# ath92/splat-renderer

Hardware: AMD Instinct MI355X
Metric: Msplats/sec (higher is better)
Workload: dtype f32

## Files before the change

### include/splat.h

```cpp
#ifndef SPLAT_H
#define SPLAT_H

#include <stddef.h>
#include <stdint.h>

#ifdef __cplusplus
extern "C" {
#endif

#define SPLAT_ABI_VERSION 3

#define SPLAT_OK 0
#define SPLAT_ERR_INVALID (-1)
#define SPLAT_ERR_HIP (-2)
#define SPLAT_ERR_OOM (-3)
#define SPLAT_ERR_CAPACITY (-4)
#define SPLAT_ERR_STATE (-5)
#define SPLAT_ERR_NO_DEVICE (-6)
#define SPLAT_ERR_COMM (-7)
#define SPLAT_ERR_RETRY (-8)

typedef struct splat_ctx splat_ctx;
typedef struct splat_sorter splat_sorter;
typedef struct splat_binner splat_binner;
// ... 17 lines not shown

int splat_ctx_create(int device_ordinal, splat_ctx **out);
int splat_ctx_create_on_stream(int device_ordinal, void *hip_stream, splat_ctx **out);
void splat_ctx_destroy(splat_ctx *ctx);
const char *splat_last_error(splat_ctx *ctx);
int splat_sync(splat_ctx *ctx);
int splat_abi_version(void);
int splat_set_timing(splat_ctx *ctx, int enabled);
#define SPLAT_TIMING_COUNT_ENTRIES 0x80000000u
int splat_set_timing_stages(splat_ctx *ctx, uint32_t stage_mask);
int splat_set_timing_sampling(splat_ctx *ctx, uint32_t every);
int splat_stage_time_ms(splat_ctx *ctx, int stage, float *ms);
int splat_stage_time_stats(splat_ctx *ctx, int stage, uint32_t *samples, double *total_ms);
int splat_timing_consumed(splat_ctx *ctx, uint64_t *staged, uint64_t *consumed);

int splat_buf_alloc(splat_ctx *ctx, size_t bytes, void **dptr);
int splat_buf_free(splat_ctx *ctx, void *dptr);
int splat_buf_upload(splat_ctx *ctx, void *dst_dptr, const void *src_host, size_t bytes);
int splat_buf_download(splat_ctx *ctx, void *dst_host, const void *src_dptr, size_t bytes);
int splat_buf_zero(splat_ctx *ctx, void *dptr, size_t bytes);
int splat_buf_copy(splat_ctx *ctx, void *dst_dptr, const void *src_dptr, size_t bytes);

int splat_update_props(splat_ctx *ctx, const void *positions, const void *curvature, uint32_t n,
                       void *props);
int splat_update_props_planes(splat_ctx *ctx, const void *positions, const void *curvature, uint32_t n,
                              void *pos_radius, void *color_opacity);
int splat_props_to_planes(splat_ctx *ctx, const void *props, uint32_t n, void *pos_radius, void *color_opacity);

int splat_project(splat_ctx *ctx, const float *uniforms, const void *pos_radius,
                  uint32_t pr_stride_vec4, uint32_t n, void *projected, void *keys, void *payload,
                  uint32_t n_padded);

int splat_extract_keys(splat_ctx *ctx, const void *projected, uint32_t n, uint32_t n_padded,
                       void *keys, void *payload);

int splat_sort_create(splat_ctx *ctx, uint32_t capacity, splat_sorter **out);
void splat_sort_destroy(splat_sorter *s);
uint32_t splat_sort_capacity(const splat_sorter *s);
void *splat_sort_keys(splat_sorter *s);
void *splat_sort_payload(splat_sorter *s);
int splat_sort_run(splat_sorter *s, uint32_t n, uint32_t bit_begin, uint32_t bit_end);
void *splat_sort_sorted_payload(splat_sorter *s);
void *splat_sort_sorted_keys(splat_sorter *s);
int splat_probe_lds_atomic_order(splat_ctx *ctx, uint64_t *mismatches);
int splat_sort_set_mode(splat_sorter *s, int mode);
int splat_rank_status(splat_ctx *ctx, int *policy, int *atomics_ordered, uint32_t *order_faults);
#ifdef SPLAT_TEST_HOOKS
int splat_debug_inject_order_fault(splat_ctx *ctx, uint32_t tile, uint32_t position);
int splat_debug_set_tile_order(splat_ctx *ctx, const void *order_dptr);
int splat_debug_set_tile_sort_order(splat_ctx *ctx, const void *order_dptr);
int splat_debug_rerun_tile_sort(splat_ctx *ctx, splat_binner *binner);
int splat_debug_tile_sort_launches(splat_ctx *ctx, uint32_t *launches);
int splat_debug_lds_rate(splat_ctx *ctx, int kind, uint32_t workgroups_per_cu, uint32_t iters, float *ms);
#endif
int splat_composite_forget_history(splat_ctx *ctx);
int splat_composite_options(splat_ctx *ctx, int kernel, int ahead, int predict);

int splat_scan_u32(splat_ctx *ctx, const void *in, void *out, uint32_t n, void *total_dptr);

int splat_bin_create(splat_ctx *ctx, uint32_t tile_size, splat_binner **out);
void splat_bin_destroy(splat_binner *b);
int splat_bin_run(splat_binner *b, const void *projected, uint32_t n_splats, const void *sorted,
                  uint32_t n_sorted, uint32_t width, uint32_t height, uint32_t tile_row0,
                  uint32_t tile_row1);
uint32_t splat_bin_tile_size(const splat_binner *b);
int splat_bin_counts(splat_binner *b, void **dptr);
int splat_bin_offsets(splat_binner *b, void **dptr);
int splat_bin_indices(splat_binner *b, void **dptr);
int splat_bin_total(splat_binner *b, uint64_t *total_pairs);
#define SPLAT_FRAME_ORDER_DEFAULT (-1)
#define SPLAT_FRAME_SORT_FIRST 0
#define SPLAT_FRAME_TILE_FIRST 1
int splat_bin_set_frame_order(splat_binner *b, int order);
int splat_bin_dims(splat_binner *b, uint32_t *ntx, uint32_t *nty);

int splat_validate_tile_order(splat_ctx *ctx, const void *projected, const void *tile_offsets,
                              uint32_t num_tiles, const void *tile_indices, uint64_t total_pairs,
                              uint64_t *violations_host);

#define SPLAT_COMPOSITE_FRONT_TO_BACK 0
#define SPLAT_COMPOSITE_REFERENCE_LITERAL 1
#define SPLAT_RECORDS_PROJECTED 0
#define SPLAT_RECORDS_COMPACT 1
#define SPLAT_RECORDS_DISC48 2
#define SPLAT_RECORDS_LIT32 3
#define SPLAT_FOOTPRINT_ISOTROPIC 0
#define SPLAT_FOOTPRINT_DISC 1
#define SPLAT_FOOTPRINT_ELLIPSOID 2
typedef struct splat_composite_cfg {
    uint32_t mode;
    uint32_t early_out;
    uint32_t tile_size;
    uint32_t tile_row0;
    uint32_t tile_row1;
    uint32_t record_format;
    uint32_t prelit;
    uint32_t footprint;
} splat_composite_cfg;
int splat_lit_colors(splat_ctx *ctx, const void *color_opacity, uint32_t color_stride_vec4,
                     const void *normals, uint32_t normal_stride_vec4, uint32_t n, void *lit);
int splat_composite(splat_ctx *ctx, const splat_composite_cfg *cfg, const void *color_opacity,
                    uint32_t color_stride_vec4, const void *normals, uint32_t normal_stride_vec4,
                    const void *projected, const void *tile_indices, const void *tile_counts,
                    const void *tile_offsets, uint32_t width, uint32_t height, void *out_rgba8,
                    void *out_rgba32f, void *consumed_dptr);

// ... 245 lines not shown
```

### splat_renderer_amd/_lib.py

```python
import ctypes as C
import os

_HERE = os.path.dirname(os.path.abspath(__file__))
LIB_PATH = os.environ.get("SPLAT_LIB_PATH") or os.path.join(_HERE, "libsplat_hip.so")

OK = 0
ERR_NAMES = {-1: "INVALID", -2: "HIP", -3: "OOM", -4: "CAPACITY", -5: "STATE", -6: "NO_DEVICE", -7: "COMM", -8: "RETRY"}
ERR_CAPACITY, ERR_RETRY = -4, -8
RENDER_AGAIN = (ERR_CAPACITY, ERR_RETRY)

STAGE_PROJECT, STAGE_SORT, STAGE_BIN, STAGE_COMPOSITE, STAGE_EXCHANGE, STAGE_BIN_SCATTER, STAGE_BIN_PASS2, STAGE_BIN_TILE_SORT = range(8)
STAGE_NAMES = ("project", "sort", "bin", "composite", "exchange", "bin_scatter", "bin_second_pass", "bin_tile_sort")
TIMING_COUNT_ENTRIES = 0x80000000
MODE_FRONT_TO_BACK, MODE_REFERENCE_LITERAL = 0, 1
RECORDS_PROJECTED, RECORDS_COMPACT, RECORDS_DISC48, RECORDS_LIT32 = 0, 1, 2, 3
FOOTPRINT_ISOTROPIC, FOOTPRINT_DISC, FOOTPRINT_ELLIPSOID = 0, 1, 2
U32_MAX = 0xFFFFFFFF


class SplatError(RuntimeError):
    def __init__(self, code, msg):
        super().__init__(f"libsplat_hip error {ERR_NAMES.get(code, code)}: {msg}")
        self.code = code

# ... 128 lines not shown
    "splat_bin_destroy": (None, [_vp]),
    "splat_bin_run": (_i, [_vp, _vp, _u32, _vp, _u32, _u32, _u32, _u32, _u32]),
    "splat_bin_tile_size": (_u32, [_vp]),
    "splat_bin_counts": (_i, [_vp, _pvp]),
    "splat_bin_offsets": (_i, [_vp, _pvp]),
    "splat_bin_indices": (_i, [_vp, _pvp]),
    "splat_bin_total": (_i, [_vp, C.POINTER(C.c_uint64)]),
    "splat_bin_set_frame_order": (_i, [_vp, _i]),
    "splat_bin_dims": (_i, [_vp, C.POINTER(_u32), C.POINTER(_u32)]),
    "splat_validate_tile_order": (_i, [_vp, _vp, _vp, _u32, _vp, C.c_uint64, C.POINTER(C.c_uint64)]),
    "splat_lit_colors": (_i, [_vp, _vp, _u32, _vp, _u32, _u32, _vp]),
    "splat_composite": (_i, [_vp, C.POINTER(CompositeCfg), _vp, _u32, _vp, _u32, _vp, _vp, _vp, _vp, _u32, _u32,
                             _vp, _vp, _vp]),
    "splat_render_frame": (_i, [_vp, _vp, _vp, C.POINTER(CompositeCfg), C.POINTER(C.c_float), _vp, _vp, _u32, _u32,
                                _u32, _vp, _vp, _vp]),
    "splat_render_frame_planes": (_i, [_vp, _vp, _vp, C.POINTER(CompositeCfg), C.POINTER(C.c_float), _vp, _vp, _vp, _u32,
                                       _u32, _u32, _vp, _vp, _vp]),
    "splat_composite_aov": (_i, [_vp, C.POINTER(CompositeCfg), _vp, _u32, _vp, _u32, _vp, _vp, _vp, _vp, _u32, _u32,
                                 _vp, _vp, _vp, C.POINTER(Aov)]),
    "splat_render_frame_aov": (_i, [_vp, _vp, _vp, C.POINTER(CompositeCfg), C.POINTER(C.c_float), _vp, _vp, _u32, _u32,
                                    _u32, _vp, _vp, _vp, C.POINTER(Aov)]),
    "splat_render_frame_planes_aov": (_i, [_vp, _vp, _vp, C.POINTER(CompositeCfg), C.POINTER(C.c_float), _vp, _vp, _vp,
                                           _u32, _u32, _u32, _vp, _vp, _vp, C.POINTER(Aov)]),
    "splat_project_slice": (_i, [_vp, C.POINTER(C.c_float), _vp, _u32, _u32, _u32, _vp]),
    "splat_project_slice_compact": (_i, [_vp, C.POINTER(C.c_float), _vp, _u32, _u32, _u32, _vp]),
    "splat_project_slice_disc": (_i, [_vp, C.POINTER(C.c_float), _vp, _u32, _vp, _u32, _u32, _u32, _vp]),
    "splat_expand_compact": (_i, [_vp, _vp, _u32, _u32, _vp]),
    "splat_band_frame": (_i, [_vp, _vp, _vp, C.POINTER(CompositeCfg), _vp, _vp, _vp, _u32, _u32, _u32, _vp, _vp, _vp]),
    "splat_band_settle": (_i, [_vp, _vp, _vp, C.POINTER(_u32), C.POINTER(C.c_uint64)]),
    "splat_band_kept": (_i, [_vp, _vp, C.POINTER(_u32)]),
    "splat_band_keys": (_i, [_vp, _vp, _vp, _u32, _u32, _u32, _u32, _u32, _u32, C.POINTER(_u32)]),
    "splat_sdf_gradients": (_i, [_vp, _vp, _u32, _vp, _u32, _vp]),
    "splat_sdf_update_positions": (_i, [_vp, _vp, _vp, _u32, _vp]),
    "splat_sdf_scale_factors": (_i, [_vp, _vp, _u32, _vp, _u32, _vp]),
    "splat_sdf_curvature": (_i, [_vp, _vp, _vp, _u32, _vp]),
    "splat_sdf_seed_positions": (_i, [_vp, C.POINTER(C.c_float), C.POINTER(C.c_float), _u32, C.c_uint64, _vp]),
    "splat_sdf_generate": (_i, [_vp, _vp, _u32, C.POINTER(C.c_float), C.POINTER(C.c_float), C.c_uint64, _vp, _u32, _u32, _vp, _vp, _vp, _vp]),
    "splat_point_frame": (_i, [_vp, _vp, C.POINTER(C.c_float), _vp, _u32, _vp, _u32, _vp, _u32, _u32, _u32, _u32, _vp, _vp, _vp, _vp]),
    "splat_comm_unique_id": (_i, [_vp]),
    "splat_comm_init": (_i, [_vp, _i, _i, _vp, _pvp]),
    "splat_comm_destroy": (None, [_vp]),
    "splat_comm_rank": (_i, [_vp, C.POINTER(_i), C.POINTER(_i)]),
    "splat_comm_count": (_i, [_vp, C.POINTER(_i), C.POINTER(_i)]),
    "splat_allgather_records": (_i, [_vp, _vp, _vp, _vp, _sz]),
}
COMM_ID_BYTES = 128
HOOK_SIGNATURES = {
    "splat_debug_inject_order_fault": (_i, [_vp, _u32, _u32]),
    "splat_debug_set_tile_order": (_i, [_vp, _vp]),
    "splat_debug_set_tile_sort_order": (_i, [_vp, _vp]),
    "splat_debug_rerun_tile_sort": (_i, [_vp, _vp]),
    "splat_debug_tile_sort_launches": (_i, [_vp, C.POINTER(_u32)]),
    "splat_debug_lds_rate": (_i, [_vp, _i, _u32, _u32, C.POINTER(C.c_float)]),
}
HOOKS_LIB_PATH = os.path.join(_HERE, "libsplat_hip_hooks.so")

_lib = None


class _Bound:

    def __getattr__(self, name):
        if name in HOOK_SIGNATURES:
            raise AttributeError(f"libsplat_hip: {name} is a test hook: the shipped library does not carry it; run with "
                                 f"SPLAT_LIB_PATH={HOOKS_LIB_PATH} (the -DSPLAT_TEST_HOOKS build)")
        raise AttributeError(f"libsplat_hip: {name} is not declared in splat_renderer_amd._lib.SIGNATURES")


def load():
    global _lib
    if _lib is not None:
        return _lib
    if not os.path.exists(LIB_PATH):
        raise ImportError(
            f"{LIB_PATH} not found: build it with `python -c 'import __graft_entry__ as g; g.build()'` "
            "(hipcc --offload-arch=gfx950). splat_renderer_amd has no CPU fallback.")
    dll = C.CDLL(LIB_PATH)
    lib = _Bound()
    for name, (res, args) in SIGNATURES.items():
        fn = getattr(dll, name)
        fn.restype = res
        fn.argtypes = args
        setattr(lib, name, fn)
    lib.has_hooks = hasattr(dll, "splat_debug_inject_order_fault")
    if lib.has_hooks:
        for name, (res, args) in HOOK_SIGNATURES.items():
            fn = getattr(dll, name)
            fn.restype = res
            fn.argtypes = args
            setattr(lib, name, fn)
    lib._dll = dll
    _lib = lib
    return lib


def check(rc, ctx=None):
    if rc != OK:
        msg = load().splat_last_error(ctx)
        raise SplatError(rc, msg.decode("utf-8", "replace") if msg else "")
    return rc
```

### splat_renderer_amd/csrc/project.hip

```cpp
#include "common.h"
#include "variant.h"
#include "tile_range.h"
#include "block_scan.h"
#include "disc.h"
#include "ellipsoid.h"
#include "shade.h"

struct FrameUniforms {
    float m[16];
    float eye[3];
    float time;
    float w, h;
};

__device__ __forceinline__ void to_screen(const FrameUniforms &u, float x, float y, float z, float &sx, float &sy) {
    float cx = ((u.m[0] * x + u.m[4] * y) + u.m[8] * z) + u.m[12];
    float cy = ((u.m[1] * x + u.m[5] * y) + u.m[9] * z) + u.m[13];
    float cw = ((u.m[3] * x + u.m[7] * y) + u.m[11] * z) + u.m[15];
    float nx = cx / cw, ny = cy / cw;
    sx = ((nx + 1.0f) * 0.5f) * u.w;
    sy = ((1.0f - ny) * 0.5f) * u.h;
}

__device__ __forceinline__ uint32_t depth_key(float depth) {
    uint32_t bits = __float_as_uint(depth);
    uint32_t mask = ((bits >> 31) == 1u) ? 0xffffffffu : 0x80000000u;
    return bits ^ mask;
}

__device__ __forceinline__ float4 project_centre(const FrameUniforms &u, float4 pr) {
    float x = pr.x, y = pr.y, z = pr.z, radius = pr.w;
    float dx = x - u.eye[0], dy = y - u.eye[1], dz = z - u.eye[2];
    float depth = sqrtf((dx * dx + dy * dy) + dz * dz);
    float scx, scy;
    to_screen(u, x, y, z, scx, scy);
    float max_d2 = 0.0f;
#pragma unroll
    for (int k = 0; k < 6; ++k) {
        float ox = (k == 0) ? radius : (k == 1) ? -radius : 0.0f;
        float oy = (k == 2) ? radius : (k == 3) ? -radius : 0.0f;
        float oz = (k == 4) ? radius : (k == 5) ? -radius : 0.0f;
        float sx, sy;
        to_screen(u, x + ox, y + oy, z + oz, sx, sy);
        float ex = scx - sx, ey = scy - sy;
        max_d2 = fmaxf(max_d2, ex * ex + ey * ey);
    }
    const float max_r = sqrtf(max_d2);
    return make_float4(scx, scy, max_r, depth);
}

struct DiscIO {
    const float4 *normals;
    uint32_t normal_stride;
    float4 *discs;
    uint32_t disc_stride;
    EllIO ell;
};

template <bool BALL>
__device__ __forceinline__ bool cannot_reach_band(const FrameUniforms &u, float4 pr, float r, const BinParams &bp) {
    const float *m = u.m;
    const float cx = ((m[0] * pr.x + m[4] * pr.y) + m[8] * pr.z) + m[12];
    const float cy = ((m[1] * pr.x + m[5] * pr.y) + m[9] * pr.z) + m[13];
    const float cw = ((m[3] * pr.x + m[7] * pr.y) + m[11] * pr.z) + m[15];
    const float ax = r * (BALL ? 1.001f * __builtin_amdgcn_sqrtf((m[0] * m[0] + m[4] * m[4]) + m[8] * m[8])
                               : fmaxf(fmaxf(fabsf(m[0]), fabsf(m[4])), fabsf(m[8])));
    const float ay = r * (BALL ? 1.001f * __builtin_amdgcn_sqrtf((m[1] * m[1] + m[5] * m[5]) + m[9] * m[9])
                               : fmaxf(fmaxf(fabsf(m[1]), fabsf(m[5])), fabsf(m[9])));
    const float aw = r * (BALL ? 1.001f * __builtin_amdgcn_sqrtf((m[3] * m[3] + m[7] * m[7]) + m[11] * m[11])
                               : fmaxf(fmaxf(fabsf(m[3]), fabsf(m[7])), fabsf(m[11])));
    const float den = cw - aw;
    if (!(cw > 0.0f) || !(den > 0.0f)) return false;
    const float icw = __builtin_amdgcn_rcpf(cw), iden = __builtin_amdgcn_rcpf(den);
    const float ndx = cx * icw, ndy = cy * icw;
    const float bx = (0.5f * u.w) * (ax + fabsf(ndx) * aw) * iden, by = (0.5f * u.h) * (ay + fabsf(ndy) * aw) * iden;
    const float reach = __builtin_amdgcn_sqrtf(bx * bx + by * by) * (1.5f * 1.001f) + 1.0f;
    const float scy = ((1.0f - ndy) * 0.5f) * u.h;
    const float ts = (float)bp.tile;
    return (scy + reach < (float)bp.row0 * ts - 2.0f) || (scy - reach > (float)bp.row1 * ts + 2.0f);
}

struct SplatIn {
    float4 pr, col, nrm, scl, rot;
};
template <bool DISC, bool LIT, bool ELL = false>
__device__ __forceinline__ SplatIn load_splat(const float4 *__restrict__ pos_radius, uint32_t stride_vec4, uint32_t i, const DiscIO &dio,
                                              const LitIO &lio) {
    SplatIn s;
    s.pr = pos_radius[(size_t)i * stride_vec4];
    s.col = s.nrm = s.scl = s.rot = make_float4(0.0f, 0.0f, 0.0f, 0.0f);
    if (ELL) {
        s.scl = dio.ell.scales[(size_t)i * dio.ell.scale_stride];
        s.rot = dio.ell.rotations[(size_t)i * dio.ell.rot_stride];
    } else if (DISC) s.nrm = dio.normals[(size_t)i * dio.normal_stride];
    if (LIT) {
        s.col = lio.color[(size_t)i * lio.color_stride];
        if (!lio.prelit) s.nrm = lio.normals[(size_t)i * lio.normal_stride];
    }
    return s;
}

template <bool WITH_KEYS, bool WITH_RANGE, bool DISC, bool LIT = false, bool WIDE = false, bool ELL = false>
__device__ __forceinline__ uint32_t project_one(const FrameUniforms &u, const SplatIn &in, uint32_t i, uint32_t index_base,
                                                float4 *__restrict__ projected, uint32_t *__restrict__ keys,
                                                uint32_t *__restrict__ payload, uint32_t *__restrict__ range32, const BinParams &bp,
                                                const DiscIO &dio, const LitIO &lio = LitIO{}, uint32_t kslot = 0xffffffffu) {
    const uint32_t ks = kslot == 0xffffffffu ? i : kslot;
    float4 a, b;
    float depth;
    if (DISC) {
        const float4 pr = in.pr;
        const DiscRecord d = ELL ? ellipsoid_record(u.m, u.w, u.h, pr, in.scl, in.rot) : disc_record(u.m, u.w, u.h, pr, in.nrm);
        dio.discs[(size_t)i * dio.disc_stride] = d.a;
        dio.discs[(size_t)i * dio.disc_stride + 1] = d.b;
        const float dx = pr.x - u.eye[0], dy = pr.y - u.eye[1], dz = pr.z - u.eye[2];
        depth = sqrtf((dx * dx + dy * dy) + dz * dz);
        if (LIT) {
            const float4 lc = (ELL || lio.prelit) ? in.col : lit_color(in.col, in.nrm);
            dio.discs[(size_t)i * dio.disc_stride + 2] = make_float4(lc.x, lc.y, lc.z, depth);
        }
        disc_bounds(d, a);
        b = make_float4(depth, 0.5f * fmaxf(a.z - a.x, a.w - a.y), __uint_as_float(index_base + i), 0.0f);
    } else {
        const float4 c = project_centre(u, in.pr);
        const float scx = c.x, scy = c.y, max_r = c.z;
        depth = c.w;
        float padded = max_r * 1.5f;
        a = make_float4(scx - padded, scy - padded, scx + padded, scy + padded);
        b = make_float4(depth, max_r, __uint_as_float(index_base + i), 0.0f);
        if (LIT) {
            lio.records[(size_t)i * 2] = c;
            lio.records[(size_t)i * 2 + 1] = lio.prelit ? in.col : lit_color(in.col, in.nrm);
        }
    }
    if ((!DISC && !LIT) || projected) {
        projected[(size_t)i * 2] = a;
        projected[(size_t)i * 2 + 1] = b;
    }
    if (WITH_KEYS) {
        keys[ks] = depth_key(depth);
        if (payload) payload[ks] = index_base + i;
    }
    uint32_t packed = 1u;
    if (WITH_RANGE) {
        uint32_t tx0, tx1, ty0, ty1;
        const bool ok = tile_range(a, bp.width, bp.height, bp.tile, bp.ntx, bp.nty, bp.row0, bp.row1, tx0, tx1, ty0, ty1);
        if (WIDE) {
            reinterpret_cast<uint2 *>(range32)[ks] = pack_range_wide(ok, tx0, tx1, ty0, ty1);
        } else {
            packed = pack_range32(ok, tx0, tx1, ty0, ty1);
            range32[ks] = packed;
        }
    }
    return packed;
}

__global__ __launch_bounds__(256) void k_project_compact(FrameUniforms u, const float4 *__restrict__ pos_radius, uint32_t stride_vec4,
                                                         uint32_t n, float4 *__restrict__ records16) {
    const uint32_t i = blockIdx.x * 256u + threadIdx.x;
    if (i < n) records16[i] = project_centre(u, pos_radius[(size_t)i * stride_vec4]);
}

__global__ __launch_bounds__(256) void k_project_disc48(FrameUniforms u, const float4 *__restrict__ pos_radius, uint32_t stride_vec4,
                                                        const float4 *__restrict__ normals, uint32_t normal_stride, uint32_t n,
                                                        float4 *__restrict__ records48) {
    const uint32_t i = blockIdx.x * 256u + threadIdx.x;
    if (i >= n) return;
    const float4 pr = pos_radius[(size_t)i * stride_vec4];
    const DiscRecord d = disc_record(u.m, u.w, u.h, pr, normals[(size_t)i * normal_stride]);
    const float dx = pr.x - u.eye[0], dy = pr.y - u.eye[1], dz = pr.z - u.eye[2];
    records48[(size_t)i * 3] = d.a;
    records48[(size_t)i * 3 + 1] = d.b;
    records48[(size_t)i * 3 + 2] = make_float4(sqrtf((dx * dx + dy * dy) + dz * dz), 0.0f, 0.0f, 0.0f);
}

__global__ __launch_bounds__(256) void k_expand_compact(const float4 *__restrict__ records16, uint32_t n, uint32_t index_base,
                                                        float4 *__restrict__ projected) {
    const uint32_t i = blockIdx.x * 256u + threadIdx.x;
    if (i >= n) return;
    const float4 c = records16[i];
    const float padded = c.z * 1.5f;
    projected[(size_t)i * 2] = make_float4(c.x - padded, c.y - padded, c.x + padded, c.y + padded);
    projected[(size_t)i * 2 + 1] = make_float4(c.w, c.z, __uint_as_float(index_base + i), 0.0f);
}

template <bool WITH_KEYS, bool WITH_RANGE, bool DISC, bool LIT = false, bool ELL = false>
__global__ __launch_bounds__(256) void k_project(FrameUniforms u, const float4 *__restrict__ pos_radius,
                                                 uint32_t stride_vec4, uint32_t n, uint32_t n_padded, uint32_t index_base,
                                                 float4 *__restrict__ projected, uint32_t *__restrict__ keys,
                                                 uint32_t *__restrict__ payload, uint32_t *__restrict__ range32, BinParams bp,
                                                 DiscIO dio, LitIO lio) {
    uint32_t i = blockIdx.x * 256u + threadIdx.x;
    if (i >= n) {
        if (WITH_KEYS && i < n_padded) {
            keys[i] = 0xffffffffu;
            if (payload) payload[i] = 0xffffffffu;
        }
        return;
    }
    const SplatIn in = load_splat<DISC, LIT, ELL>(pos_radius, stride_vec4, i, dio, lio);
    project_one<WITH_KEYS, WITH_RANGE, DISC, LIT, false, ELL>(u, in, i, index_base, projected, keys, payload, range32, bp, dio, lio);
}

template <bool DISC, bool LIT, bool ELL = false>
__global__ __launch_bounds__(256) void k_project_wide(FrameUniforms u, const float4 *__restrict__ pos_radius, uint32_t stride_vec4,
                                                      uint32_t n, uint32_t n_padded, float4 *__restrict__ projected,
                                                      uint32_t *__restrict__ keys, uint2 *__restrict__ range_wide, BinParams bp,
                                                      DiscIO dio, LitIO lio) {
    const uint32_t i = blockIdx.x * 256u + threadIdx.x;
    if (i >= n) {
        if (i < n_padded) keys[i] = 0xffffffffu;
        return;
    }
    const SplatIn in = load_splat<DISC, LIT, ELL>(pos_radius, stride_vec4, i, dio, lio);
    project_one<true, true, DISC, LIT, true, ELL>(u, in, i, 0, projected, keys, nullptr, reinterpret_cast<uint32_t *>(range_wide), bp, dio,
                                                  lio);
}

template <bool DISC, bool LIT, uint32_t PER, uint32_t AHEAD = 1, bool ELL = false>
__global__ __launch_bounds__(256) void k_project_hist(FrameUniforms u, const float4 *__restrict__ pos_radius, uint32_t stride_vec4,
                                                      uint32_t n, uint32_t n_padded, float4 *__restrict__ projected,
                                                      uint32_t *__restrict__ keys, uint32_t *__restrict__ range32, BinParams bp,
                                                      TfHistOut ho, DiscIO dio, LitIO lio) {
    __shared__ uint32_t lh[4][256];
    __shared__ uint32_t wsum[4];
    const uint32_t tid = threadIdx.x, w = tid >> 6;
    const uint32_t blk = xcd_block_of(blockIdx.x, ho.xcd_per);
    if (blk * (PER * 256u) >= n_padded) return;
    SplatIn in[PER];
#pragma unroll
    for (uint32_t k = 0; k < AHEAD; ++k) {
        const uint32_t i = blk * (PER * 256u) + k * 256u + tid;
        if (i < n) in[k] = load_splat<DISC, LIT, ELL>(pos_radius, stride_vec4, i, dio, lio);
    }
    if (blk == 0 && tid == 0) *ho.overflow_flag = 0;
    for (uint32_t j = tid; j < 4 * 256; j += 256) (&lh[0][0])[j] = 0;
    __syncthreads();
    uint32_t local = 0;
#pragma unroll
    for (uint32_t k = 0; k < PER; ++k) {
        if (k + AHEAD < PER) {
            const uint32_t i = blk * (PER * 256u) + (k + AHEAD) * 256u + tid;
            if (i < n) in[k + AHEAD] = load_splat<DISC, LIT, ELL>(pos_radius, stride_vec4, i, dio, lio);
        }
        const uint32_t i = blk * (PER * 256u) + k * 256u + tid;
        if (i >= n) {
            if (i < n_padded) keys[i] = 0xffffffffu;
            continue;
        }
        const uint32_t r = project_one<true, true, DISC, LIT, false, ELL>(u, in[k], i, 0, projected, keys, nullptr, range32, bp, dio, lio);
        const TileRect t = unpack_range32(r);
        if (t.empty()) continue;
        local += hist_add_rect(lh[w], t, bp.ntx, ho.mask);
    }
    local = wave_sum(local);
    if ((tid & 63) == 0) wsum[w] = local;
    __syncthreads();
    if (blk < ho.num_parts) {
        hist_flush<4>(lh, ho.hist, ho.num_parts, blk, ho.mask);
        if (tid == 0) ho.blocksums[blk] = wsum[0] + wsum[1] + wsum[2] + wsum[3];
    }
}

template <bool DISC, bool LIT>
__global__ __launch_bounds__(256) void k_project_hist_band(FrameUniforms u, const float4 *__restrict__ pos_radius, uint32_t stride_vec4,
                                                           uint32_t n, uint32_t n_padded, float4 *__restrict__ projected,
                                                           uint32_t *__restrict__ keys, uint32_t *__restrict__ range32, BinParams bp,
                                                           TfHistOut ho, DiscIO dio, LitIO lio) {
    __shared__ uint32_t lh[4][256];
    __shared__ uint32_t wsum[4];
    __shared__ uint32_t s_list[1024];
    __shared__ uint32_t s_count;
    const uint32_t tid = threadIdx.x, w = tid >> 6, lane = tid & 63;
    if (blockIdx.x == 0 && tid == 0) *ho.overflow_flag = 0;
    if (tid == 0) s_count = 0;
    for (uint32_t j = tid; j < 4 * 256; j += 256) (&lh[0][0])[j] = 0;
    __syncthreads();
#pragma unroll
    for (uint32_t k = 0; k < 4; ++k) {
        const uint32_t i = blockIdx.x * 1024u + k * 256u + tid;
        bool keep = false;
        if (i < n) {
            const float4 pr = pos_radius[(size_t)i * stride_vec4];
            float r = fabsf(pr.w);
            if (DISC) {
                const float4 nr = dio.normals[(size_t)i * dio.normal_stride];
                r *= fmaxf(1.0f, 1.001f * __builtin_amdgcn_sqrtf((nr.x * nr.x + nr.y * nr.y) + nr.z * nr.z));
            }
            keep = !cannot_reach_band<DISC>(u, pr, r, bp);
            if (!keep) {
                keys[i] = 0xffffffffu;
                range32[i] = 1u;
            }
        } else if (i < n_padded) {
            keys[i] = 0xffffffffu;
        }
        const unsigned long long m = __ballot(keep);
        uint32_t base = 0;
        if (lane == 0 && m) base = atomicAdd(&s_count, (uint32_t)__popcll(m));
        base = (uint32_t)__shfl((int)base, 0);
        if (keep) s_list[base + __builtin_amdgcn_mbcnt_hi((uint32_t)(m >> 32), __builtin_amdgcn_mbcnt_lo((uint32_t)m, 0))] = i;
    }
    __syncthreads();
// ... 147 lines not shown

__global__ __launch_bounds__(256) void k_sampling_rate_max(FrameUniforms u, float focal_px, float near, float margin, const float4 *__restrict__ pos,
                                                           uint32_t stride_vec4, uint32_t n, float *__restrict__ rate) {
    const uint32_t i = blockIdx.x * 256u + threadIdx.x;
    if (i >= n) return;
    const float4 p = pos[(size_t)i * stride_vec4];
    const float cw = ((u.m[3] * p.x + u.m[7] * p.y) + u.m[11] * p.z) + u.m[15];
    float scx, scy;
    to_screen(u, p.x, p.y, p.z, scx, scy);
    const float lo_x = (-margin) * u.w, hi_x = (1.0f + margin) * u.w, lo_y = (-margin) * u.h, hi_y = (1.0f + margin) * u.h;
    if (cw > near && scx >= lo_x && scx <= hi_x && scy >= lo_y && scy <= hi_y) rate[i] = fmaxf(rate[i], focal_px / cw);
}

__global__ __launch_bounds__(256) void k_extract_keys(const float4 *__restrict__ projected, uint32_t n, uint32_t n_padded,
                                                      uint32_t *__restrict__ keys, uint32_t *__restrict__ payload) {
    uint32_t i = blockIdx.x * 256u + threadIdx.x;
    if (i >= n_padded) return;
    if (i >= n) {
        keys[i] = 0xffffffffu;
        payload[i] = 0xffffffffu;
        return;
    }
    float depth = reinterpret_cast<const float *>(projected)[(size_t)i * 8 + 4];
    keys[i] = depth_key(depth);
    payload[i] = i;
}

__global__ __launch_bounds__(256) void k_update_props(const float4 *__restrict__ positions, const float4 *__restrict__ curvature,
                                                      uint32_t n, float4 *__restrict__ props) {
    uint32_t i = blockIdx.x * 256u + threadIdx.x;
    if (i >= n) return;
    float4 p = positions[i], c = curvature[i];
    props[(size_t)i * 2] = make_float4(p.x, p.y, p.z, 0.04f);
    props[(size_t)i * 2 + 1] = make_float4(fabsf(c.x) * 0.8f + 0.2f, fabsf(c.y) * 0.8f + 0.2f, fabsf(c.z) * 0.8f + 0.2f, 1.0f);
}

__global__ __launch_bounds__(256) void k_update_props_planes(const float4 *__restrict__ positions,
                                                             const float4 *__restrict__ curvature, uint32_t n,
                                                             float4 *__restrict__ pos_radius, float4 *__restrict__ color_opacity) {
    uint32_t i = blockIdx.x * 256u + threadIdx.x;
    if (i >= n) return;
    float4 p = positions[i], c = curvature[i];
    pos_radius[i] = make_float4(p.x, p.y, p.z, 0.04f);
    color_opacity[i] = make_float4(fabsf(c.x) * 0.8f + 0.2f, fabsf(c.y) * 0.8f + 0.2f, fabsf(c.z) * 0.8f + 0.2f, 1.0f);
}

__global__ __launch_bounds__(256) void k_props_to_planes(const float4 *__restrict__ props, uint32_t n,
                                                         float4 *__restrict__ pos_radius, float4 *__restrict__ color_opacity) {
    uint32_t i = blockIdx.x * 256u + threadIdx.x;
    if (i >= n) return;
    pos_radius[i] = props[(size_t)i * 2];
    color_opacity[i] = props[(size_t)i * 2 + 1];
}

static void load_uniforms(FrameUniforms &u, const float *uniforms) {
    for (int i = 0; i < 16; ++i) u.m[i] = uniforms[i];
    u.eye[0] = uniforms[16]; u.eye[1] = uniforms[17]; u.eye[2] = uniforms[18];
    u.time = uniforms[19]; u.w = uniforms[20]; u.h = uniforms[21];
}

int project_launch(splat_ctx *ctx, const ProjectArgs &a) {
    const uint32_t pr_stride_vec4 = a.pr_stride_vec4, n = a.n, index_base = a.index_base, n_padded = a.n_padded;
    const uint32_t normal_stride_vec4 = a.normal_stride_vec4;
    void *const projected = a.projected, *const keys = a.keys, *const payload = a.payload, *const discs = a.discs;
    uint32_t *const range32 = a.range32;
    uint2 *const range_wide = a.range_wide;
    const BinParams *const bp = a.bp;
    const TfHistOut *const hist_out = a.hist_out;
    const LitIO *const lit = a.lit;
    const EllIO *const ell = a.ell;
    FrameUniforms u;
    load_uniforms(u, a.uniforms);
    const uint32_t work = keys ? n_padded : n;
    if (work == 0) return SPLAT_OK;
    BinParams none = {0, 0, 1, 0, 0, 0, 0};
    const float4 *src = (const float4 *)a.pos_radius + (size_t)index_base * pr_stride_vec4;
    const bool disc = discs != nullptr;
    const bool el = disc && ell != nullptr;
    if (el && hist_out && bp && bp->skip_outside)
        return ctx_fail(ctx, SPLAT_ERR_INVALID, "project_launch: the ellipsoid footprint has no band projector");
    const bool with_lit = lit && lit->records && !disc, disc_lit = lit && lit->records && disc;
    if ((with_lit || disc_lit) && !(keys && (range32 || range_wide) && !payload && index_base == 0))
        return ctx_fail(ctx, SPLAT_ERR_INVALID, "project_launch: lit records are written by the frame's projector only");
    DiscIO dio = {(disc && !el) ? (const float4 *)a.normals + (size_t)index_base * normal_stride_vec4 : nullptr, normal_stride_vec4,
                  (float4 *)discs, disc_lit ? 3u : 2u, EllIO{}};
    if (el) {
        dio.ell = *ell;
        dio.ell.scales += (size_t)index_base * ell->scale_stride;
        dio.ell.rotations += (size_t)index_base * ell->rot_stride;
    }
    const LitIO lio = (with_lit || disc_lit) ? *lit : LitIO{};
    stage_begin(ctx, SPLAT_STAGE_PROJECT);
    const dim3 block(256);
    const bool lit_out = with_lit || disc_lit;
    const bool frame_keys = keys && !payload && index_base == 0;
    bool ok = false;
    if (hist_out && frame_keys && range32 && bp->skip_outside) {
        TfHistOut ho = *hist_out;
        if (hist_out->cidx) {
            const XcdGrid xg = xcd_grid(ho.num_parts);
            ho.xcd_per = xg.xcd_per;
            const dim3 grid(xg.grid);
            ok = variant_dispatch(
                [&](auto d, auto l) {
                    launch_kernel(ctx, NO_STAGE, k_project_hist_bandc<d.value, l.value>, grid, dim3(PBC_THREADS), u, src, pr_stride_vec4, n,
                                  (float4 *)projected, (uint32_t *)keys, range32, *bp, ho, dio, lio);
                    return true;
                },
                disc, lit_out);
        } else {
            ok = variant_dispatch(
                [&](auto d, auto l) {
                    launch_kernel(ctx, NO_STAGE, k_project_hist_band<d.value, l.value>, dim3(div_up(work, 1024)), block, u, src, pr_stride_vec4, n,
                                  n_padded, (float4 *)projected, (uint32_t *)keys, range32, *bp, ho, dio, lio);
                    return true;
                },
                disc, lit_out);
        }
    } else if (hist_out && frame_keys && range32) {
        TfHistOut ho = *hist_out;
        const bool small = hist_out->block == TF_BLOCK_SMALL;
        const uint32_t blocks = div_up(work, small ? 256u : 1024u);
        const XcdGrid xg = xcd_grid(blocks);
        ho.xcd_per = xg.xcd_per;
        const dim3 grid(xg.grid);
        ok = variant_dispatch(
            [&](auto d, auto l, auto per, auto e) {
                if constexpr (d.value || !e.value) {
                    launch_kernel(ctx, NO_STAGE, k_project_hist<d.value, l.value, per.value, 1, e.value>, grid, block, u, src, pr_stride_vec4, n,
                                  n_padded, (float4 *)projected, (uint32_t *)keys, range32, *bp, ho, dio, lio);
                    return true;
                } else return false;
            },
            disc, lit_out, OneOf<1, 4>{small ? 1 : 4}, el);
    } else if (frame_keys && range_wide) {
        ok = variant_dispatch(
            [&](auto d, auto l, auto e) {
                if constexpr (d.value || !e.value) {
                    launch_kernel(ctx, NO_STAGE, k_project_wide<d.value, l.value, e.value>, dim3(div_up(work, 256)), block, u, src, pr_stride_vec4, n,
                                  n_padded, (float4 *)projected, (uint32_t *)keys, range_wide, *bp, dio, lio);
                    return true;
                } else return false;
            },
            disc, lit_out, el);
    } else {
        const bool with_keys = keys != nullptr, with_range = keys && range32;
        ok = variant_dispatch(
            [&](auto k, auto r, auto d, auto l, auto e) {
                if constexpr ((k.value || !r.value) && (r.value || !l.value) && (d.value || !e.value)) {
                    launch_kernel(ctx, NO_STAGE, k_project<k.value, r.value, d.value, l.value, e.value>, dim3(div_up(work, 256)), block, u, src,
                                  pr_stride_vec4, n, with_keys ? n_padded : n, index_base, (float4 *)projected, (uint32_t *)keys,
                                  (uint32_t *)payload, with_range ? range32 : nullptr, with_range ? *bp : none, dio, lio);
                    return true;
                } else return false;
            },
            with_keys, with_range, disc, with_range && lit_out, el);
    }
    if (!ok) return ctx_fail(ctx, SPLAT_ERR_INVALID, "project_launch: no kernel for this footprint and these outputs");
    LAUNCH_CHECK(ctx, "k_project");
    stage_end(ctx, SPLAT_STAGE_PROJECT);
    return SPLAT_OK;
}

int project_ellipsoid_aa_launch(splat_ctx *ctx, const ProjectAaArgs &a) {
    const uint32_t work = a.keys ? a.n_padded : a.n;
    if (work == 0) return SPLAT_OK;
    FrameUniforms u;
    load_uniforms(u, a.uniforms);
    const AaIO aa = {a.rho_out, (const float4 *)a.color_opacity, a.color_stride_vec4, (float4 *)a.color_opacity_out};
    if (a.timed) stage_begin(ctx, SPLAT_STAGE_PROJECT);
    hipLaunchKernelGGL(k_project_ellipsoid_aa, dim3(div_up(work, 256)), dim3(256), 0, ctx->stream, u, (const float4 *)a.positions, a.pos_stride_vec4,
                       a.n, work, (float4 *)a.projected, (float4 *)a.records, (uint32_t *)a.keys, (uint32_t *)a.payload, *a.ell, aa);
    LAUNCH_CHECK(ctx, "k_project_ellipsoid_aa");
    if (a.timed) stage_end(ctx, SPLAT_STAGE_PROJECT);
    return SPLAT_OK;
}

extern "C" {

int splat_project(splat_ctx *ctx, const float *uniforms, const void *pos_radius, uint32_t pr_stride_vec4, uint32_t n,
                  void *projected, void *keys, void *payload, uint32_t n_padded) {
    if (!ctx) return ctx_fail(nullptr, SPLAT_ERR_INVALID, "ctx is NULL");
    ARG_CHECK(ctx, uniforms && (n == 0 || (pos_radius && projected)));
    ARG_CHECK(ctx, pr_stride_vec4 >= 1);
    ARG_CHECK(ctx, (keys == nullptr) == (payload == nullptr));
    ARG_CHECK(ctx, keys == nullptr || n_padded >= n);
    ARG_CHECK(ctx, (((uintptr_t)pos_radius | (uintptr_t)projected) & 15) == 0);
// ... 119 lines not shown
int splat_expand_compact(splat_ctx *ctx, const void *records16, uint32_t n, uint32_t index_base, void *projected) {
    if (!ctx) return ctx_fail(nullptr, SPLAT_ERR_INVALID, "ctx is NULL");
    ARG_CHECK(ctx, n == 0 || (records16 && projected));
    ARG_CHECK(ctx, (((uintptr_t)records16 | (uintptr_t)projected) & 15) == 0);
    if (n == 0) return SPLAT_OK;
    hipLaunchKernelGGL(k_expand_compact, dim3(div_up(n, 256)), dim3(256), 0, ctx->stream, (const float4 *)records16, n, index_base,
                       (float4 *)projected);
    LAUNCH_CHECK(ctx, "k_expand_compact");
    return SPLAT_OK;
}

int splat_extract_keys(splat_ctx *ctx, const void *projected, uint32_t n, uint32_t n_padded, void *keys, void *payload) {
    if (!ctx) return ctx_fail(nullptr, SPLAT_ERR_INVALID, "ctx is NULL");
    ARG_CHECK(ctx, keys && payload && (n == 0 || projected) && n_padded >= n);
    if (n_padded == 0) return SPLAT_OK;
    hipLaunchKernelGGL(k_extract_keys, dim3(div_up(n_padded, 256)), dim3(256), 0, ctx->stream, (const float4 *)projected, n,
                       n_padded, (uint32_t *)keys, (uint32_t *)payload);
    LAUNCH_CHECK(ctx, "k_extract_keys");
    return SPLAT_OK;
}

int splat_update_props(splat_ctx *ctx, const void *positions, const void *curvature, uint32_t n, void *props) {
    if (!ctx) return ctx_fail(nullptr, SPLAT_ERR_INVALID, "ctx is NULL");
    ARG_CHECK(ctx, n == 0 || (positions && curvature && props));
    if (n == 0) return SPLAT_OK;
    hipLaunchKernelGGL(k_update_props, dim3(div_up(n, 256)), dim3(256), 0, ctx->stream, (const float4 *)positions,
                       (const float4 *)curvature, n, (float4 *)props);
    LAUNCH_CHECK(ctx, "k_update_props");
    return SPLAT_OK;
}

int splat_update_props_planes(splat_ctx *ctx, const void *positions, const void *curvature, uint32_t n, void *pos_radius,
                              void *color_opacity) {
    if (!ctx) return ctx_fail(nullptr, SPLAT_ERR_INVALID, "ctx is NULL");
    ARG_CHECK(ctx, n == 0 || (positions && curvature && pos_radius && color_opacity));
    if (n == 0) return SPLAT_OK;
    hipLaunchKernelGGL(k_update_props_planes, dim3(div_up(n, 256)), dim3(256), 0, ctx->stream, (const float4 *)positions,
                       (const float4 *)curvature, n, (float4 *)pos_radius, (float4 *)color_opacity);
    LAUNCH_CHECK(ctx, "k_update_props_planes");
    return SPLAT_OK;
}

int splat_props_to_planes(splat_ctx *ctx, const void *props, uint32_t n, void *pos_radius, void *color_opacity) {
    if (!ctx) return ctx_fail(nullptr, SPLAT_ERR_INVALID, "ctx is NULL");
    ARG_CHECK(ctx, n == 0 || (props && pos_radius && color_opacity));
    ARG_CHECK(ctx, (((uintptr_t)props | (uintptr_t)pos_radius | (uintptr_t)color_opacity) & 15) == 0);
    if (n == 0) return SPLAT_OK;
    hipLaunchKernelGGL(k_props_to_planes, dim3(div_up(n, 256)), dim3(256), 0, ctx->stream, (const float4 *)props, n, (float4 *)pos_radius,
                       (float4 *)color_opacity);
    LAUNCH_CHECK(ctx, "k_props_to_planes");
    return SPLAT_OK;
}

}
```

### splat_renderer_amd/csrc/tile_range.h

```cpp
#pragma once
#include <hip/hip_runtime.h>
#include <stdint.h>

__device__ __forceinline__ bool tile_range(float4 bounds, uint32_t width, uint32_t height, uint32_t tile, uint32_t ntx,
                                           uint32_t nty, uint32_t row0, uint32_t row1, uint32_t &tx0, uint32_t &tx1,
                                           uint32_t &ty0, uint32_t &ty1) {
    if (isnan(bounds.x) || isnan(bounds.y) || isnan(bounds.z) || isnan(bounds.w)) return false;
    float min_x = fmaxf(bounds.x, 0.0f), min_y = fmaxf(bounds.y, 0.0f);
    float max_x = fminf(bounds.z, (float)width), max_y = fminf(bounds.w, (float)height);
    if (min_x >= max_x || min_y >= max_y) return false;
    if ((tile & (tile - 1)) == 0) {
        const float inv = 1.0f / (float)tile;
        float a = floorf(min_x * inv), b = fminf(floorf(max_x * inv), (float)(ntx - 1u));
        float c = floorf(min_y * inv), d = fminf(floorf(max_y * inv), (float)(nty - 1u));
        if (a > b || c > d) return false;
        tx0 = (uint32_t)a; tx1 = (uint32_t)b; ty0 = (uint32_t)c; ty1 = (uint32_t)d;
    } else {
        double ts = (double)tile;
        double a = floor((double)min_x / ts), b = fmin(floor((double)max_x / ts), (double)ntx - 1.0);
        double c = floor((double)min_y / ts), d = fmin(floor((double)max_y / ts), (double)nty - 1.0);
        if (a > b || c > d) return false;
        tx0 = (uint32_t)a; tx1 = (uint32_t)b; ty0 = (uint32_t)c; ty1 = (uint32_t)d;
    }
    if (ty0 < row0) ty0 = row0;
    if (row1 == 0) return false;
    if (ty1 > row1 - 1) ty1 = row1 - 1;
    return ty0 <= ty1;
}


__device__ __forceinline__ uint32_t pack_range32(bool ok, uint32_t tx0, uint32_t tx1, uint32_t ty0, uint32_t ty1) {
    return ok ? (tx0 | (tx1 << 8) | (ty0 << 16) | (ty1 << 24)) : 1u;
}
struct TileRect {
    uint32_t tx0, tx1, ty0, ty1;
    __device__ __forceinline__ bool empty() const { return tx0 > tx1 || ty0 > ty1; }
};
__device__ __forceinline__ TileRect unpack_range32(uint32_t r) { return {r & 0xffu, (r >> 8) & 0xffu, (r >> 16) & 0xffu, r >> 24}; }

__device__ __forceinline__ uint2 pack_range_wide(bool ok, uint32_t tx0, uint32_t tx1, uint32_t ty0, uint32_t ty1) {
    return ok ? make_uint2(tx0 | (tx1 << 16), ty0 | (ty1 << 16)) : make_uint2(1u, 1u);
}

__device__ __forceinline__ uint32_t range32_hits(uint32_t r) {
    const TileRect t = unpack_range32(r);
    return t.empty() ? 0u : (t.tx1 - t.tx0 + 1) * (t.ty1 - t.ty0 + 1);
}
__device__ __forceinline__ uint32_t range_hits(uint2 r) {
    const uint32_t tx0 = r.x & 0xffffu, tx1 = r.x >> 16, ty0 = r.y & 0xffffu, ty1 = r.y >> 16;
    return (tx0 > tx1 || ty0 > ty1) ? 0u : (tx1 - tx0 + 1) * (ty1 - ty0 + 1);
}

__device__ __forceinline__ uint32_t hist_add_rect(uint32_t *wave_hist, TileRect t, uint32_t ntx, uint32_t mask) {
    for (uint32_t ty = t.ty0; ty <= t.ty1; ++ty)
        for (uint32_t tx = t.tx0; tx <= t.tx1; ++tx) atomicAdd(&wave_hist[(ty * ntx + tx) & mask], 1u);
    return (t.tx1 - t.tx0 + 1) * (t.ty1 - t.ty0 + 1);
}
```

Before: 15610.

## Use shared reciprocal division for projection when operands lie in safe range

```diff
diff --git a/include/splat.h b/include/splat.h
--- a/include/splat.h
+++ b/include/splat.h
@@ -93,6 +93,7 @@
 int splat_debug_rerun_tile_sort(splat_ctx *ctx, splat_binner *binner);
 int splat_debug_tile_sort_launches(splat_ctx *ctx, uint32_t *launches);
 int splat_debug_lds_rate(splat_ctx *ctx, int kind, uint32_t workgroups_per_cu, uint32_t iters, float *ms);
+int splat_debug_shared_rcp_div(splat_ctx *ctx, const void *triples, uint32_t n, void *out);
 #endif
 int splat_composite_forget_history(splat_ctx *ctx);
 int splat_composite_options(splat_ctx *ctx, int kernel, int ahead, int predict);
diff --git a/splat_renderer_amd/_lib.py b/splat_renderer_amd/_lib.py
--- a/splat_renderer_amd/_lib.py
+++ b/splat_renderer_amd/_lib.py
@@ -204,6 +204,7 @@
     "splat_debug_rerun_tile_sort": (_i, [_vp, _vp]),
     "splat_debug_tile_sort_launches": (_i, [_vp, C.POINTER(_u32)]),
     "splat_debug_lds_rate": (_i, [_vp, _i, _u32, _u32, C.POINTER(C.c_float)]),
+    "splat_debug_shared_rcp_div": (_i, [_vp, _vp, _u32, _vp]),
 }
 HOOKS_LIB_PATH = os.path.join(_HERE, "libsplat_hip_hooks.so")
 
diff --git a/splat_renderer_amd/csrc/project.hip b/splat_renderer_amd/csrc/project.hip
--- a/splat_renderer_amd/csrc/project.hip
+++ b/splat_renderer_amd/csrc/project.hip
@@ -1,6 +1,7 @@
 #include "common.h"
 #include "variant.h"
 #include "tile_range.h"
+#include "shared_rcp_div.h"
 #include "block_scan.h"
 #include "disc.h"
 #include "ellipsoid.h"
@@ -13,35 +14,64 @@
     float w, h;
 };
 
-__device__ __forceinline__ void to_screen(const FrameUniforms &u, float x, float y, float z, float &sx, float &sy) {
-    float cx = ((u.m[0] * x + u.m[4] * y) + u.m[8] * z) + u.m[12];
-    float cy = ((u.m[1] * x + u.m[5] * y) + u.m[9] * z) + u.m[13];
-    float cw = ((u.m[3] * x + u.m[7] * y) + u.m[11] * z) + u.m[15];
-    float nx = cx / cw, ny = cy / cw;
-    sx = ((nx + 1.0f) * 0.5f) * u.w;
-    sy = ((1.0f - ny) * 0.5f) * u.h;
-}
-
 __device__ __forceinline__ uint32_t depth_key(float depth) {
     uint32_t bits = __float_as_uint(depth);
     uint32_t mask = ((bits >> 31) == 1u) ? 0xffffffffu : 0x80000000u;
     return bits ^ mask;
 }
 
+struct ClipPoint {
+    srd_float2 xy;
+    float w;
+};
+__device__ __forceinline__ ClipPoint to_clip(const FrameUniforms &u, float x, float y, float z) {
+    ClipPoint c;
+    c.xy.x = ((u.m[0] * x + u.m[4] * y) + u.m[8] * z) + u.m[12];
+    c.xy.y = ((u.m[1] * x + u.m[5] * y) + u.m[9] * z) + u.m[13];
+    c.w = ((u.m[3] * x + u.m[7] * y) + u.m[11] * z) + u.m[15];
+    return c;
+}
+__device__ __forceinline__ void ndc_to_screen(const FrameUniforms &u, srd_float2 ndc, float &sx, float &sy) {
+    sx = ((ndc.x + 1.0f) * 0.5f) * u.w;
+    sy = ((1.0f - ndc.y) * 0.5f) * u.h;
+}
+__device__ __forceinline__ void to_screen(const FrameUniforms &u, float x, float y, float z, float &sx, float &sy) {
+    const ClipPoint c = to_clip(u, x, y, z);
+    ndc_to_screen(u, srd_float2{c.xy.x / c.w, c.xy.y / c.w}, sx, sy);
+}
+
 __device__ __forceinline__ float4 project_centre(const FrameUniforms &u, float4 pr) {
     float x = pr.x, y = pr.y, z = pr.z, radius = pr.w;
     float dx = x - u.eye[0], dy = y - u.eye[1], dz = z - u.eye[2];
     float depth = sqrtf((dx * dx + dy * dy) + dz * dz);
-    float scx, scy;
-    to_screen(u, x, y, z, scx, scy);
-    float max_d2 = 0.0f;
+    ClipPoint c[7];
+    c[0] = to_clip(u, x, y, z);
 #pragma unroll
     for (int k = 0; k < 6; ++k) {
         float ox = (k == 0) ? radius : (k == 1) ? -radius : 0.0f;
         float oy = (k == 2) ? radius : (k == 3) ? -radius : 0.0f;
         float oz = (k == 4) ? radius : (k == 5) ? -radius : 0.0f;
+        c[k + 1] = to_clip(u, x + ox, y + oy, z + oz);
+    }
+    SrdWindow win;
+#pragma unroll
+    for (int k = 0; k < 7; ++k) win.add(c[k].xy.x, c[k].xy.y, c[k].w);
+    srd_float2 ndc[7];
+    if (win.inside()) {
+#pragma unroll
+        for (int k = 0; k < 7; ++k) ndc[k] = srd_divide2(c[k].xy, c[k].w);
+    } else {
+        asm volatile("" ::: "memory");
+#pragma unroll
+        for (int k = 0; k < 7; ++k) ndc[k] = srd_float2{c[k].xy.x / c[k].w, c[k].xy.y / c[k].w};
+    }
+    float scx, scy;
+    ndc_to_screen(u, ndc[0], scx, scy);
+    float max_d2 = 0.0f;
+#pragma unroll
+    for (int k = 1; k < 7; ++k) {
         float sx, sy;
-        to_screen(u, x + ox, y + oy, z + oz, sx, sy);
+        ndc_to_screen(u, ndc[k], sx, sy);
         float ex = scx - sx, ey = scy - sy;
         max_d2 = fmaxf(max_d2, ex * ex + ey * ey);
     }
@@ -100,7 +130,7 @@
     return s;
 }
 
-template <bool WITH_KEYS, bool WITH_RANGE, bool DISC, bool LIT = false, bool WIDE = false, bool ELL = false>
+template <bool WITH_KEYS, bool WITH_RANGE, bool DISC, bool LIT = false, bool WIDE = false, bool ELL = false, bool POW2 = false>
 __device__ __forceinline__ uint32_t project_one(const FrameUniforms &u, const SplatIn &in, uint32_t i, uint32_t index_base,
                                                 float4 *__restrict__ projected, uint32_t *__restrict__ keys,
                                                 uint32_t *__restrict__ payload, uint32_t *__restrict__ range32, const BinParams &bp,
@@ -122,6 +152,8 @@
         disc_bounds(d, a);
         b = make_float4(depth, 0.5f * fmaxf(a.z - a.x, a.w - a.y), __uint_as_float(index_base + i), 0.0f);
     } else {
+        float4 lc = make_float4(0.0f, 0.0f, 0.0f, 0.0f);
+        if (LIT) lc = lio.prelit ? in.col : lit_color(in.col, in.nrm);
         const float4 c = project_centre(u, in.pr);
         const float scx = c.x, scy = c.y, max_r = c.z;
         depth = c.w;
@@ -130,7 +162,7 @@
         b = make_float4(depth, max_r, __uint_as_float(index_base + i), 0.0f);
         if (LIT) {
             lio.records[(size_t)i * 2] = c;
-            lio.records[(size_t)i * 2 + 1] = lio.prelit ? in.col : lit_color(in.col, in.nrm);
+            lio.records[(size_t)i * 2 + 1] = lc;
         }
     }
     if ((!DISC && !LIT) || projected) {
@@ -144,7 +176,7 @@
     uint32_t packed = 1u;
     if (WITH_RANGE) {
         uint32_t tx0, tx1, ty0, ty1;
-        const bool ok = tile_range(a, bp.width, bp.height, bp.tile, bp.ntx, bp.nty, bp.row0, bp.row1, tx0, tx1, ty0, ty1);
+        const bool ok = tile_range<POW2>(a, bp.width, bp.height, bp.tile, bp.ntx, bp.nty, bp.row0, bp.row1, tx0, tx1, ty0, ty1);
         if (WIDE) {
             reinterpret_cast<uint2 *>(range32)[ks] = pack_range_wide(ok, tx0, tx1, ty0, ty1);
         } else {
@@ -217,7 +249,7 @@
                                                   lio);
 }
 
-template <bool DISC, bool LIT, uint32_t PER, uint32_t AHEAD = 1, bool ELL = false>
+template <bool DISC, bool LIT, uint32_t PER, uint32_t AHEAD = 1, bool ELL = false, bool POW2 = false>
 __global__ __launch_bounds__(256) void k_project_hist(FrameUniforms u, const float4 *__restrict__ pos_radius, uint32_t stride_vec4,
                                                       uint32_t n, uint32_t n_padded, float4 *__restrict__ projected,
                                                       uint32_t *__restrict__ keys, uint32_t *__restrict__ range32, BinParams bp,
@@ -248,7 +280,7 @@
             if (i < n_padded) keys[i] = 0xffffffffu;
             continue;
         }
-        const uint32_t r = project_one<true, true, DISC, LIT, false, ELL>(u, in[k], i, 0, projected, keys, nullptr, range32, bp, dio, lio);
+        const uint32_t r = project_one<true, true, DISC, LIT, false, ELL, POW2>(u, in[k], i, 0, projected, keys, nullptr, range32, bp, dio, lio);
         const TileRect t = unpack_range32(r);
         if (t.empty()) continue;
         local += hist_add_rect(lh[w], t, bp.ntx, ho.mask);
@@ -502,6 +534,23 @@
     pos_radius[i] = props[(size_t)i * 2];
     color_opacity[i] = props[(size_t)i * 2 + 1];
 }
+
+#ifdef SPLAT_TEST_HOOKS
+__global__ __launch_bounds__(256) void k_debug_shared_rcp_div(const float *__restrict__ triples, uint32_t n, uint32_t *__restrict__ out) {
+    const uint32_t i = blockIdx.x * 256u + threadIdx.x;
+    if (i >= n) return;
+    const float nx = triples[(size_t)i * 3], ny = triples[(size_t)i * 3 + 1], d = triples[(size_t)i * 3 + 2];
+    SrdWindow win;
+    win.add(nx, ny, d);
+    const srd_float2 plain = {nx / d, ny / d};
+    srd_float2 fast = plain;
+    if (win.inside()) fast = srd_divide2(srd_float2{nx, ny}, d);
+    uint32_t *o = out + (size_t)i * 5;
+    o[0] = __float_as_uint(fast.x), o[1] = __float_as_uint(fast.y);
+    o[2] = __float_as_uint(plain.x), o[3] = __float_as_uint(plain.y);
+    o[4] = win.inside() ? 1u : 0u;
+}
+#endif
 
 static void load_uniforms(FrameUniforms &u, const float *uniforms) {
     for (int i = 0; i < 16; ++i) u.m[i] = uniforms[i];
@@ -575,14 +624,14 @@
         ho.xcd_per = xg.xcd_per;
         const dim3 grid(xg.grid);
         ok = variant_dispatch(
-            [&](auto d, auto l, auto per, auto e) {
+            [&](auto d, auto l, auto per, auto e, auto p2) {
                 if constexpr (d.value || !e.value) {
-                    launch_kernel(ctx, NO_STAGE, k_project_hist<d.value, l.value, per.value, 1, e.value>, grid, block, u, src, pr_stride_vec4, n,
-                                  n_padded, (float4 *)projected, (uint32_t *)keys, range32, *bp, ho, dio, lio);
+                    launch_kernel(ctx, NO_STAGE, k_project_hist<d.value, l.value, per.value, 1, e.value, p2.value>, grid, block, u, src,
+                                  pr_stride_vec4, n, n_padded, (float4 *)projected, (uint32_t *)keys, range32, *bp, ho, dio, lio);
                     return true;
                 } else return false;
             },
-            disc, lit_out, OneOf<1, 4>{small ? 1 : 4}, el);
+            disc, lit_out, OneOf<1, 4>{small ? 1 : 4}, el, (bp->tile & (bp->tile - 1)) == 0);
     } else if (frame_keys && range_wide) {
         ok = variant_dispatch(
             [&](auto d, auto l, auto e) {
@@ -808,4 +857,16 @@
     return SPLAT_OK;
 }
 
-}
+#ifdef SPLAT_TEST_HOOKS
+int splat_debug_shared_rcp_div(splat_ctx *ctx, const void *triples, uint32_t n, void *out) {
+    if (!ctx) return ctx_fail(nullptr, SPLAT_ERR_INVALID, "ctx is NULL");
+    ARG_CHECK(ctx, n == 0 || (triples && out));
+    ARG_CHECK(ctx, (((uintptr_t)triples | (uintptr_t)out) & 3) == 0);
+    if (n == 0) return SPLAT_OK;
+    hipLaunchKernelGGL(k_debug_shared_rcp_div, dim3(div_up(n, 256)), dim3(256), 0, ctx->stream, (const float *)triples, n, (uint32_t *)out);
+    LAUNCH_CHECK(ctx, "k_debug_shared_rcp_div");
+    return SPLAT_OK;
+}
+#endif
+
+}
diff --git a/splat_renderer_amd/csrc/shared_rcp_div.h b/splat_renderer_amd/csrc/shared_rcp_div.h
--- /dev/null
+++ b/splat_renderer_amd/csrc/shared_rcp_div.h
@@ -0,0 +1,30 @@
+#pragma once
+#include <hip/hip_runtime.h>
+#include <stdint.h>
+
+typedef float srd_float2 __attribute__((ext_vector_type(2)));
+
+constexpr uint32_t SRD_LO_BITS = 0x2f800000u;
+constexpr uint32_t SRD_HI_BITS = 0x4f800000u;
+
+struct SrdWindow {
+    uint32_t off = 0u, frac = 0u;
+    static __device__ __forceinline__ uint32_t key(float v) { return (__float_as_uint(v) << 1) + (0u - 2u * SRD_LO_BITS); }
+    __device__ __forceinline__ void add(float nx, float ny, float d) {
+        off = max(off, max(key(nx), max(key(ny), key(d))));
+        frac = max(frac, __float_as_uint(d) << 9);
+    }
+    __device__ __forceinline__ bool inside() const { return off <= 2u * (SRD_HI_BITS - SRD_LO_BITS) && frac != 0xfffffe00u; }
+};
+
+__device__ __forceinline__ srd_float2 srd_divide2(srd_float2 n, float d) {
+    const float r0 = __builtin_amdgcn_rcpf(d);
+    const float e = __builtin_fmaf(-d, r0, 1.0f);
+    const float r = __builtin_fmaf(e, r0, r0);
+    const srd_float2 nd = {-d, -d}, rr = {r, r};
+    const srd_float2 q0 = n * rr;
+    const srd_float2 t = __builtin_elementwise_fma(nd, q0, n);
+    const srd_float2 q1 = __builtin_elementwise_fma(t, rr, q0);
+    const srd_float2 u = __builtin_elementwise_fma(nd, q1, n);
+    return __builtin_elementwise_fma(u, rr, q1);
+}
diff --git a/splat_renderer_amd/csrc/tile_range.h b/splat_renderer_amd/csrc/tile_range.h
--- a/splat_renderer_amd/csrc/tile_range.h
+++ b/splat_renderer_amd/csrc/tile_range.h
@@ -2,6 +2,7 @@
 #include <hip/hip_runtime.h>
 #include <stdint.h>
 
+template <bool POW2 = false>
 __device__ __forceinline__ bool tile_range(float4 bounds, uint32_t width, uint32_t height, uint32_t tile, uint32_t ntx,
                                            uint32_t nty, uint32_t row0, uint32_t row1, uint32_t &tx0, uint32_t &tx1,
                                            uint32_t &ty0, uint32_t &ty1) {
@@ -9,7 +10,7 @@
     float min_x = fmaxf(bounds.x, 0.0f), min_y = fmaxf(bounds.y, 0.0f);
     float max_x = fminf(bounds.z, (float)width), max_y = fminf(bounds.w, (float)height);
     if (min_x >= max_x || min_y >= max_y) return false;
-    if ((tile & (tile - 1)) == 0) {
+    if (POW2 || (tile & (tile - 1)) == 0) {
         const float inv = 1.0f / (float)tile;
         float a = floorf(min_x * inv), b = fminf(floorf(max_x * inv), (float)(ntx - 1u));
         float c = floorf(min_y * inv), d = fminf(floorf(max_y * inv), (float)(nty - 1u));
```

Measured after the change: 15630, median of 3. Within noise of the previous version (+0.1%).
